# gnss-sdr/gnss-sdr

Measured on AMD Instinct MI355X. Metric: correlators/s, higher is better.
Workload: dtype f32; 1 GPU; GPS L1 C/A tracking, 32 channels/GPU x 400 epochs/block x 1400 blocks/step, fs=25 Msps, N=25000, 3-tap E/P/L, open-loop, 2 launches in flight (blocks alternate over that many banks and streams); the IF stream is RESIDENT in HBM before the timed region (host-to-device transfer excluded: pcie_inclusive is the end-to-end figure); channels_per_gpu=32, epochs_per_block=400, samples_per_epoch=25000, taps=3, stream_resident_bytes=643200000, parallelism=channels sharded over 1 GPU(s)

## Files before the change

### gnss-sdr_amd/_lib.py

```python
from __future__ import annotations

import ctypes as C
import os

_HERE = os.path.dirname(os.path.abspath(__file__))
LIB_PATH = os.environ.get("GSH_LIB_PATH") or os.path.join(_HERE, "libgnss_sdr_hip.so")

GSH_MAX_TAPS = 8
GSH_MAX_WIDE_TAPS = 64
GSH_OK = 0
GSH_ITEM_GR_COMPLEX, GSH_ITEM_SHORT, GSH_ITEM_BYTE = 0, 1, 2
GSH_ARRAY_MAX_ANTENNAS, GSH_ARRAY_MAX_BEAMS = 8, 8
GSH_ARRAY_PLANAR, GSH_ARRAY_INTERLEAVED = 0, 1
ERR_NAMES = {1: "GSH_ERR_INVALID", 2: "GSH_ERR_NO_DEVICE", 3: "GSH_ERR_HIP", 4: "GSH_ERR_STATE", 5: "GSH_ERR_UNSUPPORTED"}


class GshError(RuntimeError):
    def __init__(self, code: int, text: str):
        super().__init__(f"{ERR_NAMES.get(code, code)}: {text}")
        self.code = code


class CorrJob(C.Structure):
    _fields_ = [
# ... 161 lines not shown
        ("noise_power_estimation", C.c_float),
        ("n_segments", C.c_int32),
        ("last_filtered", C.c_int32),
        ("n_decided", C.c_uint64),
        ("n_blanked", C.c_uint64),
    ]


class CondNotch(C.Structure):
    _fields_ = [
        ("pfa", C.c_float),
        ("p_c_factor", C.c_float),
        ("length", C.c_int32),
        ("n_segments_est", C.c_int32),
        ("n_segments_reset", C.c_int32),
        ("n_segments_coeff", C.c_int32),
    ]


class CondNotchState(C.Structure):
    _fields_ = [
        ("thres", C.c_float),
        ("noise_pow_est", C.c_float),
        ("n_segments", C.c_int32),
        ("filter_state", C.c_int32),
        ("n_segments_coeff", C.c_int32),
        ("reserved", C.c_int32),
        ("z0", C.c_float * 2),
        ("n_decided", C.c_uint64),
        ("n_filtered", C.c_uint64),
    ]


class AcqResult(C.Structure):
    _fields_ = [
        ("index_time", C.c_uint32),
        ("index_doppler", C.c_uint32),
        ("doppler_hz", C.c_int32),
        ("acq_delay_samples", C.c_float),
        ("peak", C.c_float),
        ("input_power", C.c_float),
        ("second_peak", C.c_float),
        ("test_statistics", C.c_float),
    ]


_P = C.c_void_p
_F = C.POINTER(C.c_float)
_I16 = C.POINTER(C.c_int16)
_I8 = C.POINTER(C.c_int8)
SYMBOLS = {
    "gsh_abi_version": (C.c_int, []),
    "gsh_device_count": (C.c_int, []),
    "gsh_probe_read_bandwidth": (C.c_int, [C.c_int, C.c_uint64, C.c_int, C.POINTER(C.c_double)]),
    "gsh_last_error": (C.c_char_p, []),
    "gsh_device_name": (C.c_int, [C.c_int, C.c_char_p, C.c_size_t]),
    "gsh_mcorr_create": (C.c_int, [C.c_int, C.POINTER(_P)]),
    "gsh_mcorr_destroy": (None, [_P]),
    "gsh_mcorr_init": (C.c_int, [_P, C.c_int, C.c_int]),
    "gsh_mcorr_set_local_code_and_taps": (C.c_int, [_P, C.c_int, _F, _F]),
    "gsh_mcorr_set_input_output_vectors": (C.c_int, [_P, _F, _F]),
    "gsh_mcorr_set_high_dynamics_resampler": (C.c_int, [_P, C.c_int]),
    "gsh_mcorr_carrier_wipeoff_multicorrelator_resampler": (C.c_int, [_P] + [C.c_float] * 6 + [C.c_int]),
    "gsh_mcorr_carrier_wipeoff_multicorrelator_resampler6": (C.c_int, [_P] + [C.c_float] * 5 + [C.c_int]),
    "gsh_mcorr_free": (C.c_int, [_P]),
    "gsh_mcorr16_create": (C.c_int, [C.c_int, C.POINTER(_P)]),
    "gsh_mcorr16_destroy": (None, [_P]),
    "gsh_mcorr16_init": (C.c_int, [_P, C.c_int, C.c_int]),
    "gsh_mcorr16_set_local_code_and_taps": (C.c_int, [_P, C.c_int, _I16, _F]),
    "gsh_mcorr16_set_input_output_vectors": (C.c_int, [_P, _I16, _I16]),
    "gsh_mcorr16_carrier_wipeoff_multicorrelator_resampler": (C.c_int, [_P] + [C.c_float] * 4 + [C.c_int]),
    "gsh_mcorr16_free": (C.c_int, [_P]),
    "gsh_bank16_create": (C.c_int, [C.c_int, C.c_int, C.c_int, C.POINTER(_P)]),
    "gsh_bank16_destroy": (None, [_P]),
    "gsh_bank16_set_code": (C.c_int, [_P, C.c_int, _I16, C.c_int]),
    "gsh_bank16_set_stream_host": (C.c_int, [_P, _I16, C.c_uint64]),
    "gsh_bank16_set_stream_device": (C.c_int, [_P, _P, C.c_uint64]),
    "gsh_bank16_correlate": (C.c_int, [_P, C.POINTER(Corr16Job), C.c_int, _I16]),
    "gsh_bank16_upload_jobs": (C.c_int, [_P, C.POINTER(Corr16Job), C.c_int]),
    "gsh_bank16_launch": (C.c_int, [_P]),
    "gsh_bank16_read_outputs": (C.c_int, [_P, _I16, C.c_int]),
    "gsh_bank16_time_launches": (C.c_int, [_P, C.c_int, _F]),
    "gsh_bank_create": (C.c_int, [C.c_int, C.c_int, C.c_int, C.POINTER(_P)]),
    "gsh_bank_destroy": (None, [_P]),
    "gsh_bank_set_code": (C.c_int, [_P, C.c_int, _F, C.c_int]),
    "gsh_bank_set_stream_host": (C.c_int, [_P, _F, C.c_uint64]),
    "gsh_bank_set_stream_device": (C.c_int, [_P, _P, C.c_uint64]),
    "gsh_bank_correlate": (C.c_int, [_P, C.POINTER(CorrJob), C.c_int, _F]),
    "gsh_bank_upload_jobs": (C.c_int, [_P, C.POINTER(CorrJob), C.c_int]),
    "gsh_bank_launch": (C.c_int, [_P, _P]),
    "gsh_bank_synchronize": (C.c_int, [_P]),
    "gsh_bank_read_outputs": (C.c_int, [_P, _F, C.c_int]),
    "gsh_bank_time_launches": (C.c_int, [_P, C.c_int, _F]),
    "gsh_bank_set_pair_fusion": (C.c_int, [_P, C.c_int]),
    "gsh_bank_set_splits": (C.c_int, [_P, C.c_int]),
    "gsh_bank_set_sample_base": (C.c_int, [_P, C.c_uint64]),
    "gsh_bank_set_stream_ring": (C.c_int, [_P, _P]),
    "gsh_bank_correlate_wide": (C.c_int, [_P, C.POINTER(CorrJobWide), C.c_int, _F]),
    "gsh_bank_time_launches_wide": (C.c_int, [_P, C.POINTER(CorrJobWide), C.c_int, C.c_int, _F]),
    "gsh_stream_create": (C.c_int, [C.c_int, C.c_uint64, C.c_uint32, C.POINTER(_P)]),
    "gsh_stream_destroy": (None, [_P]),
    "gsh_stream_push": (C.c_int, [_P, _P, C.c_uint64, C.c_int, C.c_int, C.POINTER(C.c_uint64)]),
    "gsh_stream_push_device": (C.c_int, [_P, _P, C.c_uint64, C.c_int, C.c_int, _P, C.POINTER(C.c_uint64)]),
    "gsh_stream_push_async": (C.c_int, [_P, _P, C.c_uint64, C.c_int, C.c_int, C.POINTER(C.c_uint64)]),
    "gsh_stream_wait": (C.c_int, [_P]),
    "gsh_stream_push_staged": (C.c_int, [_P, _P, C.c_uint64, C.c_int, C.c_int, C.POINTER(C.c_uint64)]),
# ... 178 lines not shown
```

### gnss-sdr_amd/csrc/mcorr_device.h

```cpp
#ifndef GSH_MCORR_DEVICE_H
#define GSH_MCORR_DEVICE_H

#include "gsh_internal.h"
#include <cmath>
#include <type_traits>

#ifndef GSH_MC_THREADS
#define GSH_MC_THREADS 256
#endif
#define GSH_MC_NS_CAT2(a, b) a##b
#define GSH_MC_NS_CAT(a, b) GSH_MC_NS_CAT2(a, b)
#define GSH_MC_NS GSH_MC_NS_CAT(mcdev_, GSH_MC_THREADS)

namespace gsh
{
namespace GSH_MC_NS
{
constexpr int MC_THREADS = GSH_MC_THREADS;
constexpr int MC_WAVES = MC_THREADS / 64;
constexpr int MC_MARGIN = 32;
constexpr int MC_HALF_MAX_CODE_LEN = 1024;
constexpr int MC_HALF_WORDS = 2 * (MC_HALF_MAX_CODE_LEN + 2 * MC_MARGIN);
#ifndef GSH_MC_SCAN_ALL_AT_ONCE
#define GSH_MC_SCAN_ALL_AT_ONCE 1
// ... 125 lines not shown
#undef GSH_DPP_STEP
}

__device__ __forceinline__ float readlane_f(float v, int l)
{
    return __builtin_bit_cast(float, __builtin_amdgcn_readlane(__builtin_bit_cast(int, v), l));
}

__device__ __forceinline__ int floor_to_int(float x)
{
#if GSH_MC_CVT_FLR
    int k;
    asm("v_cvt_flr_i32_f32 %0, %1" : "=v"(k) : "v"(x));
    return k;
#else
    return static_cast<int>(floorf(x));
#endif
}

__device__ __forceinline__ int raw_chip_std(float step_x_n, float shift, float rem)
{
    return floor_to_int(__fsub_rn(__fadd_rn(step_x_n, shift), rem));
}

__device__ __forceinline__ int raw_chip_hd(float step, float rate, unsigned m, float shift0, float rem)
{
    const float a = __fmul_rn(step, static_cast<float>(m));
    const float q = __fmul_rn(rate, static_cast<float>(m * m));
    return floor_to_int(__fsub_rn(__fadd_rn(__fadd_rn(a, q), shift0), rem));
}

struct JobCtx
{
    int n_total;
    int n_begin;
    int n_end;
    int n_first;
    int code_len;
    float rem_carr, phase_step, phase_rate;
    float rem_code, code_step, code_rate;
    int k_lo{0}, k_hi{-1};
    int k_off{MC_MARGIN};
    bool packed{true};
    bool runs{false};
    bool aux_on{false};
    bool aux_zero{false};
    float aux_shift{0.0f};
    int aux_code_len{1};
    int aux_k_off{MC_MARGIN};
    int aux_k_lo{0}, aux_k_hi{-1};
    const float2* seed_tab{nullptr};
    const float2* fac_tab{nullptr};
};
constexpr int FAC_B = 0;
constexpr int FAC_WH = 32;
constexpr int FAC_INC = 40;
constexpr int FAC_A = 44;
constexpr int FAC_NA = 20;
constexpr int FAC_ENTRIES = 64;
static_assert(MC_THREADS > 256 || MC_THREADS / 32 <= FAC_INC - FAC_WH, "factor table: one WH entry per 32 threads");
__host__ __device__ constexpr int packed_reseed_trips(int nch) { return (GSH_MC_RESEED + nch - 1) / nch; }
template <int NCH>
__device__ __forceinline__ void fac_table_fill(float2* __restrict__ tab, float step, float rem, int n_first, int lane)
{
    const double sd = static_cast<double>(step);
    double ph;
    if (lane < FAC_WH)
        ph = static_cast<double>(2 * lane) * sd;
    else if (lane < FAC_INC)
        ph = static_cast<double>(64 * (lane - FAC_WH)) * sd;
    else if (lane < FAC_A)
        ph = (lane == FAC_INC ? 1.0 : (lane == FAC_INC + 1 ? static_cast<double>(2 * MC_THREADS) : static_cast<double>(2 * NCH * MC_THREADS))) * sd;
    else
        {
            const long long nb = static_cast<long long>(n_first) + static_cast<long long>(2 * MC_THREADS * NCH * packed_reseed_trips(NCH)) * (lane - FAC_A);
            ph = static_cast<double>(rem) + static_cast<double>(nb) * sd;
        }
    tab[lane] = expmj(ph);
}
constexpr int SEED_B = 0;
constexpr int SEED_W = 64;
constexpr int SEED_A = 80;
constexpr int SEED_INC = 82;
constexpr int SEED_ENTRIES = 88;
__device__ __forceinline__ void seed_table_fill(float2* __restrict__ tab, float step, double rem, int lane, int which)
{
    asm volatile("" : "+v"(lane));
    const double sd = static_cast<double>(step);
    if (which == 0)
        tab[SEED_B + lane] = expmj(static_cast<double>(2 * lane) * sd);
    else if (lane < 21)
        {
            double ph;
            int at;
            if (lane < 16)
                {
                    ph = static_cast<double>(128 * lane) * sd;
                    at = SEED_W + lane;
                }
            else if (lane < 18)
                {
                    ph = rem + static_cast<double>(-(lane - 16)) * sd;
                    at = SEED_A + (lane - 16);
                }
            else
                {
// ... 441 lines not shown
                    const v2f cB = lookup(aB, aux_shp, zs, aux_koff, std::false_type{});
                    pk_fma_lo(XB0, yB0, cB);
                    pk_fma_hi(XB1, yB1, cB);
                }
        }
}

struct PairedCodes
{
    v2f p, el0, el1;
};
template <bool ZP, bool KC>
__device__ __forceinline__ PairedCodes paired_codes_of(const JobCtx& c, const float* __restrict__ tab, v2f shP, v2f shL, v2f k_step_nrem, v2f nf)
{
    typedef const __attribute__((address_space(3))) float* lds_float_ptr;
    const int koff = KC ? MC_MARGIN : c.k_off;
    const v2f a = pk_mul_slo(nf, k_step_nrem);
    auto at = [&](int k, int d) -> float {
        if constexpr (KC)
            {
                unsigned byte_addr;
                asm("v_lshlrev_b32 %0, 2, %1" : "=v"(byte_addr) : "v"(k));
                return reinterpret_cast<lds_float_ptr>(byte_addr)[MC_MARGIN + d];
            }
        else
            return tab[k + koff + d];
    };
    PairedCodes d;
    {
        const v2f u = ZP ? pk_add_shi(a, k_step_nrem) : pk_add_shi(pk_add_slo(a, shP), k_step_nrem);
        d.p.x = at(floor_to_int(u.x), 0);
        d.p.y = at(floor_to_int(u.y), 0);
    }
    {
        const v2f u = pk_add_shi(pk_add_slo(a, shL), k_step_nrem);
        const int k0 = floor_to_int(u.x), k1 = floor_to_int(u.y);
        d.el0.x = at(k0, -1);
        d.el0.y = at(k0, 0);
        d.el1.x = at(k1, -1);
        d.el1.y = at(k1, 0);
    }
    return d;
}
__device__ __forceinline__ void paired_accumulate(const PairedCodes& d, v2f y0, v2f y1, v2f (&S0)[3], v2f (&S1)[3])
{
    pk_fma_lo(S0[0], y0, d.el0);
    pk_fma_lo(S1[0], y1, d.el1);
    pk_fma_lo(S0[1], y0, d.p);
    pk_fma_hi(S1[1], y1, d.p);
    pk_fma_hi(S0[2], y0, d.el0);
    pk_fma_hi(S1[2], y1, d.el1);
}

template <int NT, bool ZP, bool AUX, int NCH, int PF, bool DER = false, bool KC = false, bool MRG = false, bool HALF = false>
__device__ __forceinline__ void run_segment_packed(const JobCtx& c, const float2* __restrict__ base, const float* __restrict__ tab,
    const float (&sh)[NT], float2 (&acc)[NT], float2* acc_aux)
{
    static_assert(NCH == 1 || NCH == 2, "one or two chunks per trip");
    static_assert(!HALF || (DER && KC && !MRG), "half-chip taps: a paired-tap flavour of the whole-code table");
    constexpr int PPC = MC_PAIRS_PER_CHUNK;
    constexpr int RESEED = packed_reseed_trips(NCH);
    constexpr int TBL = 60;
    const int tid = threadIdx.x;
    const int lane = tid & 63;
    const v2f zero = {0.0f, 0.0f};
    float2 tb_b = make_float2(1.0f, 0.0f), tb_wv = tb_b, tb_a0 = tb_b, tb_inc = tb_b, tb_w = tb_b, tb_w2 = tb_b;
    if (c.seed_tab != nullptr)
        {
            int tl = tid;
            asm volatile("" : "+v"(tl));
            const float2* __restrict__ S = c.seed_tab;
            tb_b = S[SEED_B + (tl & 63)];
            tb_wv = S[SEED_W + (tl >> 6)];
            tb_a0 = S[SEED_A + (c.n_begin - c.n_first)];
            tb_inc = S[SEED_INC];
            tb_w = S[SEED_INC + 1];
            tb_w2 = S[SEED_INC + (NCH == 2 ? 2 : 1)];
        }
    const int span = c.n_end - c.n_first;
    const int n_pairs = (span + 1) >> 1;
    const int n_full = span >> 1;
    const int odd = c.n_begin - c.n_first;
    const int n_trips_all = (n_pairs + NCH * PPC - 1) / (NCH * PPC);
    int n_trips = n_trips_all;
    if constexpr (NCH == 1 || MRG)
        {
            const int left = c.n_end - (c.n_first + 128 * (tid >> 6));
            n_trips = left <= 0 ? 0 : min(n_trips_all, (left + 2 * NCH * PPC - 1) / (2 * NCH * PPC));
            n_trips = __builtin_amdgcn_readfirstlane(n_trips);
        }
    const int first_plain = odd ? 1 : 0;
    const int last_plain = n_full / (NCH * PPC);
    constexpr int TRIP = 2 * NCH * PPC;
    unsigned lane_bytes = 16u * static_cast<unsigned>(tid);
    typedef const __attribute__((address_space(1))) char* global_bytes;
    typedef float v4f_t __attribute__((ext_vector_type(4)));
    typedef const __attribute__((address_space(1))) v4f_t* global_v4f;
    typedef const __attribute__((address_space(1))) v2f* global_v2f;
    auto trip_base = [&](int i, int byte_off) -> global_bytes {
        global_bytes ub = (global_bytes)(reinterpret_cast<const char*>(base + static_cast<long long>(i) * TRIP) + byte_off);
        asm("" : "+s"(ub));
        return ub;
    };
    auto load16 = [](global_bytes p) -> float4 {
        const v4f_t v = *(global_v4f)p;
        return make_float4(v.x, v.y, v.z, v.w);
    };
    auto load8 = [](global_bytes p) -> float2 {
        const v2f v = *(global_v2f)p;
        return make_float2(v.x, v.y);
    };
    auto lane_n0 = [&](int i) -> int {
        unsigned lb = lane_bytes;
        asm volatile("" : "+v"(lb));
        return (c.n_first + i * TRIP) + static_cast<int>(lb >> 3);
    };
// ... 643 lines not shown
                epbuf[lane] = make_float4(incl.x - tot.x, incl.y - tot.y, ph.x, ph.y);
                T = make_float2(readlane_f(incl.x, 63), readlane_f(incl.y, 63));
            }
#endif
            asm volatile("" ::: "memory");

#ifdef GSH_RUNS_SKIP3
            if (false)
#else
            if (my_t < NT)
#endif
                {
                    const int k_first = chip_of(n_lo);
                    const int count = chip_of(b - 1) - k_first;
                    if (my_j == 0)
                        {
                            const float c0 = tab[k_first + c.k_off];
                            bacc.x = fmaf(c0, T.x, bacc.x);
                            bacc.y = fmaf(c0, T.y, bacc.y);
                        }
                    for (int j = my_j; j < count; j += LT)
                        {
                            const int k = k_first + 1 + j;
                            int n = static_cast<int>(ceilf(__fmul_rn(__fadd_rn(static_cast<float>(k), est_off), inv_step)));
                            n = min(max(n, n_lo + 1), b - 1);
                            while (n > n_lo + 1 && chip_of(n - 1) >= k) n--;
                            while (n < b - 1 && chip_of(n) < k) n++;
                            const int rel = n - a;
                            const int run = rel / R, pos = rel % R;
                            const float4 ep = epbuf[run];
                            const float2 qv = ybuf[run * STRIDE + max(pos - 1, 0)];
                            float2 P = make_float2(ep.x, ep.y);
                            if (pos > 0)
                                {
                                    const float2 r = cmul(qv, make_float2(ep.z, ep.w));
                                    P.x += r.x;
                                    P.y += r.y;
                                }
                            const float d = tab[k + c.k_off] - tab[k - 1 + c.k_off];
                            bacc.x = fmaf(d, T.x - P.x, bacc.x);
                            bacc.y = fmaf(d, T.y - P.y, bacc.y);
                        }
                }
            asm volatile("" ::: "memory");
        }
#pragma unroll
    for (int t = 0; t < NT; t++)
        {
            acc[t].x += (my_t == t) ? bacc.x : 0.0f;
            acc[t].y += (my_t == t) ? bacc.y : 0.0f;
        }
}

template <int NT, int MODE, bool WRAP, bool ZP = false, bool AUX = false, bool KC = false, bool PAIRK = false, bool HALFK = false>
__device__ __forceinline__ void run_segment(const JobCtx& c, const float2* __restrict__ base, const float* __restrict__ tab,
    const float (&sh)[NT], const int (&rot)[NT], float2 (&acc)[NT], float2* acc_aux = nullptr)
{
#if GSH_MC_PACKED
    if (!WRAP && MODE == 0 && c.packed && c.n_total < (1 << 24))
        {
#ifndef GSH_MC_MERGED
#define GSH_MC_MERGED 1
#endif
#ifndef GSH_MC_MERGED_BANK
#define GSH_MC_MERGED_BANK 0
#endif
            constexpr bool MRG = GSH_MC_MERGED && (MC_THREADS > 256 || GSH_MC_MERGED_BANK);
#ifdef GSH_MC_NCH
            constexpr int NCH = (NT <= 3 && !AUX) ? GSH_MC_NCH : 1;
#else
#ifdef GSH_MC_NCH_WIDE
            constexpr int NCH = (MC_THREADS <= 256 || MRG) ? 2 : 1;
#else
            constexpr int NCH = (MC_THREADS <= 256 || (MRG && NT <= 3 && !AUX)) ? 2 : 1;
#endif
#endif
#ifdef GSH_MC_PREFETCH
            constexpr int PF = GSH_MC_PREFETCH;
#else
            constexpr int PF = (MC_THREADS <= 256) ? GSH_MC_PREFETCH_BANK : GSH_MC_PREFETCH_LOOP;
#endif
            if constexpr (PAIRK && NT == 3 && ZP && !AUX && PF == 1)
                {
                    static_assert(!HALFK || (KC && NCH == 2 && !MRG), "half-chip taps: whole-code table, two chunks per trip, four accumulator sets");
                    run_segment_packed<NT, ZP, AUX, NCH, PF, true, KC, MRG, HALFK>(c, base, tab, sh, acc, acc_aux);
                    return;
                }
            run_segment_packed<NT, ZP, AUX, NCH, PF, false, KC && !HALFK, MRG>(c, base, tab, sh, acc, acc_aux);
            return;
        }
#endif
    const int tid = threadIdx.x;
    const int span = c.n_end - c.n_first;
    const int n_pairs = (span + 1) >> 1;
    const int n_full = span >> 1;
    const int odd = c.n_begin - c.n_first;
    const int n_chunks = (n_pairs + MC_PAIRS_PER_CHUNK - 1) / MC_PAIRS_PER_CHUNK;
    const int k_full_begin = odd ? 1 : 0;
    const int k_full_end = n_full / MC_PAIRS_PER_CHUNK;
    constexpr bool HDP = mode_hd_phase(MODE);

    if (odd && n_chunks > 0)
        {
            const int pair = tid;
            if (pair < n_pairs)
                {
                    const int n0 = c.n_first + 2 * pair;
                    const float2 pa = expmj(carrier_phase<HDP>(c.rem_carr, c.phase_step, c.phase_rate, n0));
                    const float2 pb = expmj(carrier_phase<HDP>(c.rem_carr, c.phase_step, c.phase_rate, n0 + 1));
                    process_pair<NT, MODE, WRAP, true, false, AUX>(c, base, tab, sh, rot, pair, pa, pb, acc, static_cast<float>(n0), acc_aux);
                }
        }

    if (k_full_end > k_full_begin)
        {
            if (HDP)
                {
                    for (int k = k_full_begin; k < k_full_end; k++)
                        {
                            const int pair = tid + k * MC_PAIRS_PER_CHUNK;
                            const int n0 = c.n_first + 2 * pair;
                            const float2 pa = expmj(carrier_phase<true>(c.rem_carr, c.phase_step, c.phase_rate, n0));
                            const float2 pb = expmj(carrier_phase<true>(c.rem_carr, c.phase_step, c.phase_rate, n0 + 1));
                            process_pair<NT, MODE, WRAP, false, false, AUX>(c, base, tab, sh, rot, pair, pa, pb, acc, static_cast<float>(n0), acc_aux);
                        }
                }
            else
                {
                    const int k_body = k_full_begin;
                    const float2 w = expmj(static_cast<double>(2 * MC_PAIRS_PER_CHUNK) * static_cast<double>(c.phase_step));
                    const float2 inc = expmj(static_cast<double>(c.phase_step));
                    for (int kb = k_body; kb < k_full_end; kb += MC_RESEED)
                        {
                            const int cnt = min(MC_RESEED, k_full_end - kb);
                            int pair = tid + kb * MC_PAIRS_PER_CHUNK;
                            float2 pa = expmj(carrier_phase<false>(c.rem_carr, c.phase_step, 0.0f, c.n_first + 2 * pair));
                            float2 pb = cmul(pa, inc);
                            float nf0 = static_cast<float>(c.n_first + 2 * pair);
#pragma unroll 2
                            for (int i = 0; i < cnt; i++)
                                {
                                    process_pair<NT, MODE, WRAP, false, ZP, AUX>(c, base, tab, sh, rot, pair, pa, pb, acc, nf0, acc_aux);
                                    pa = cmul(pa, w);
                                    pb = cmul(pb, w);
                                    pair += MC_PAIRS_PER_CHUNK;
// ... 261 lines not shown
```

### gnss-sdr_amd/csrc/multicorrelator.hip

```cpp
#include "multicorrelator.h"
#ifdef GSH_MC_VARIANT_128
#define mcorr_kernel mcorr_kernel_t128
#define mcorr_reduce_partials mcorr_reduce_partials_t128
#endif
#include "mcorr_device.h"
#include <cmath>
#include <cstdlib>

namespace gsh
{
namespace
{
using namespace mcdev;
#ifndef GSH_MC_MIN_WAVES
#define GSH_MC_MIN_WAVES 5
#endif

#ifndef GSH_MC_RUN_LEN
#define GSH_MC_RUN_LEN 8
#endif
constexpr int MC_RUN_LEN = GSH_MC_RUN_LEN;

template <int NT, int MODE, bool AUX, bool RUNS = false, bool WIN = false, bool PAIR = false, bool HALF = false>
__global__ __launch_bounds__(MC_THREADS, ((NT <= 3 && !AUX) ? GSH_MC_MIN_WAVES : 1)) void mcorr_kernel(McorrArgs a)
{
    static_assert(!PAIR || (NT == 3 && MODE == 0 && !AUX && !RUNS), "paired taps: the plain E/P/L launch");
    static_assert(!HALF || (PAIR && !WIN), "half-chip taps: a paired-tap launch with whole-code tables");
    static_assert(!RUNS || (MODE == 0 && !AUX), "the run-based path exists for the standard mode without a fused tap");
    extern __shared__ __align__(16) float lds[];
    const unsigned lb = xcd_remap(blockIdx.x, gridDim.x);
    const int slot = static_cast<int>(lb) / a.splits;
    const int split = static_cast<int>(lb) - slot * a.splits;
    const int job = a.job_list ? a.job_list[slot] : slot;
    const gsh_corr_job& J = a.jobs[job];
    const int tid = threadIdx.x;
    const int aux_job = AUX ? a.aux[job] : -1;
    if (AUX && aux_job == -2) return;

    JobCtx c;
    c.n_total = J.n_samples;
    c.code_len = a.code_lens[J.code_slot];
    c.rem_carr = J.rem_carr_phase_rad;
    c.phase_step = J.phase_step_rad;
    c.phase_rate = J.phase_rate_step_rad;
    c.rem_code = J.rem_code_phase_chips;
    c.code_step = J.code_phase_step_chips;
    c.code_rate = J.code_phase_rate_step_chips;
    c.packed = a.packed != 0;
    c.runs = RUNS && a.packed == 2;

    int seg = (c.n_total + a.splits - 1) / a.splits;
    seg = (seg + 1) & ~1;
    c.n_begin = min(split * seg, c.n_total);
    c.n_end = min(c.n_total, c.n_begin + seg);
    unsigned long long win0 = J.sample_offset + a.sample_base;
    if (a.ring_capacity) win0 %= a.ring_capacity;
    const unsigned long long abs0 = win0 + static_cast<unsigned long long>(c.n_begin);
    const int odd = static_cast<int>(abs0 & 1ULL);
// ... 194 lines not shown
                sums[2 * NT] = acc_aux.x;
                sums[2 * NT + 1] = acc_aux.y;
            }
        wave_scan_incl_n(sums);
#pragma unroll
        for (int t = 0; t < NT; t++) acc[t] = make_float2(sums[2 * t], sums[2 * t + 1]);
        if (AUX) acc_aux = make_float2(sums[2 * NT], sums[2 * NT + 1]);
    }
    const int wave = tid >> 6;
    if ((tid & 63) == 63)
        {
#pragma unroll
            for (int t = 0; t < NT; t++) red[wave * GSH_MAX_TAPS + t] = acc[t];
            if (AUX) red[wave * GSH_MAX_TAPS + NT] = acc_aux;
        }
    __syncthreads();
    if (AUX && aux_job >= 0 && tid >= GSH_MAX_TAPS && tid < 2 * GSH_MAX_TAPS)
        {
            const int tap = tid - GSH_MAX_TAPS;
            float2 s = make_float2(0.0f, 0.0f);
            if (tap == 0)
                {
#pragma unroll
                    for (int w = 0; w < MC_WAVES; w++)
                        {
                            s.x += red[w * GSH_MAX_TAPS + NT].x;
                            s.y += red[w * GSH_MAX_TAPS + NT].y;
                        }
                }
            if (a.splits == 1)
                a.out[static_cast<size_t>(aux_job) * GSH_MAX_TAPS + tap] = s;
            else
                a.partials[(static_cast<size_t>(aux_job) * a.splits + split) * GSH_MAX_TAPS + tap] = s;
        }
    if (tid < GSH_MAX_TAPS)
        {
            float2 s = make_float2(0.0f, 0.0f);
            if (tid < NT && tid < J.n_taps)
                {
#pragma unroll
                    for (int w = 0; w < MC_WAVES; w++)
                        {
                            s.x += red[w * GSH_MAX_TAPS + tid].x;
                            s.y += red[w * GSH_MAX_TAPS + tid].y;
                        }
                }
            if (a.splits == 1)
                a.out[static_cast<size_t>(job) * GSH_MAX_TAPS + tid] = s;
            else
                a.partials[(static_cast<size_t>(job) * a.splits + split) * GSH_MAX_TAPS + tid] = s;
        }
}

__global__ __launch_bounds__(256) void mcorr_reduce_partials(const float2* __restrict__ partials, float2* __restrict__ out, int n_jobs, int splits)
{
    const int i = blockIdx.x * blockDim.x + threadIdx.x;
    if (i >= n_jobs * GSH_MAX_TAPS) return;
    const int job = i / GSH_MAX_TAPS, tap = i - job * GSH_MAX_TAPS;
    float2 s = make_float2(0.0f, 0.0f);
    for (int k = 0; k < splits; k++)
        {
            const float2 p = partials[(static_cast<size_t>(job) * splits + k) * GSH_MAX_TAPS + tap];
            s.x += p.x;
            s.y += p.y;
        }
    out[i] = s;
}

template <int NT>
int launch_nt(const McorrArgs& a, int mode, size_t lds, size_t lds_half, hipStream_t stream)
{
    const dim3 grid(static_cast<unsigned>(a.n_launch) * static_cast<unsigned>(a.splits));
    const dim3 block(MC_THREADS);
    if (a.aux != nullptr)
        {
            if constexpr (NT == 3 || NT == 5)
                {
                    GSH_REQUIRE(mode == 0, "fused jobs need the standard mode");
                    if (a.window_floats > 0)
                        hipLaunchKernelGGL((mcorr_kernel<NT, 0, true, false, true>), grid, block, lds, stream, a);
                    else
                        hipLaunchKernelGGL((mcorr_kernel<NT, 0, true>), grid, block, lds, stream, a);
                    GSH_HIP(hipGetLastError());
                    return GSH_OK;
                }
            else
                return set_error(GSH_ERR_INVALID, "fused jobs exist only for the 3- and 5-tap kernels");
        }
    switch (mode)
        {
        case 0:
#ifdef GSH_MC_RUNS_EXPERIMENT
            if constexpr (NT <= 5)
                {
                    if (a.packed == 2 && a.window_floats == 0)
                        {
                            const size_t lds_runs = lds + static_cast<size_t>(MC_WAVES) * RunsLayout<MC_RUN_LEN>::FLOATS * sizeof(float);
                            if (lds_runs <= 64 * 1024)
                                {
                                    hipLaunchKernelGGL((mcorr_kernel<NT, 0, false, true>), grid, block, lds_runs, stream, a);
                                    break;
                                }
                        }
                }
#endif
            if constexpr (NT == 3)
                {
                    if (a.pair && a.packed == 1)
                        {
                            if (a.window_floats > 0)
                                hipLaunchKernelGGL((mcorr_kernel<NT, 0, false, false, true, true>), grid, block, lds, stream, a);
                            else if (a.half && lds_half > 0 && a.code_images != nullptr)
                                hipLaunchKernelGGL((mcorr_kernel<NT, 0, false, false, false, true, true>), grid, block, lds_half, stream, a);
                            else
                                hipLaunchKernelGGL((mcorr_kernel<NT, 0, false, false, false, true>), grid, block, lds, stream, a);
                            break;
                        }
                }
            if (a.window_floats > 0)
                hipLaunchKernelGGL((mcorr_kernel<NT, 0, false, false, true>), grid, block, lds, stream, a);
            else
                hipLaunchKernelGGL((mcorr_kernel<NT, 0, false>), grid, block, lds, stream, a);
            break;
        case 1:
            hipLaunchKernelGGL((mcorr_kernel<NT, 1, false>), grid, block, lds, stream, a);
            break;
        case 2:
            hipLaunchKernelGGL((mcorr_kernel<NT, 2, false>), grid, block, lds, stream, a);
            break;
        default:
            return set_error(GSH_ERR_INVALID, "unknown correlator mode %d", mode);
        }
    GSH_HIP(hipGetLastError());
    return GSH_OK;
}
}

#ifndef GSH_MC_VARIANT_128
int mcorr_packed_default()
{
    static const int v = [] {
        const char* e = std::getenv("GSH_MC_PACKED_BODY");
        if (e != nullptr && e[0] == '0') return 0;
#ifdef GSH_MC_RUNS_EXPERIMENT
        if (e != nullptr && e[0] == '2') return 2;
#endif
        if (e != nullptr && e[0] == '3') return 3;
        return 1;
    }();
    return v;
}

int mcorr_fac_default()
{
    static const int v = [] {
        const char* e = std::getenv("GSH_MC_FAC");
        return (e != nullptr && e[0] == '0') ? 0 : 1;
    }();
    return v;
}

#endif

#ifdef GSH_MC_VARIANT_128
#define mcorr_lds_bytes_window mcorr_lds_bytes_window_t128
#define mcorr_lds_bytes_fused mcorr_lds_bytes_fused_t128
// ... 83 lines not shown
    GSH_REQUIRE(args.splits >= 1, "splits must be >= 1");
    static const int class_taps[4] = {1, 3, 5, GSH_MAX_TAPS};
    for (int c = 0; c < 4; c++)
        {
            if (plan.count[c] <= 0) continue;
            McorrArgs a = args;
            a.job_list = plan.list + plan.offset[c];
            a.n_launch = plan.count[c];
            if (!plan.aux[c]) a.aux = nullptr;
#ifndef GSH_MC_VARIANT_128
            if (use_128(a, class_taps[c], mode))
                {
                    McorrClassPlan one = plan;
                    for (int o = 0; o < 4; o++)
                        if (o != c) one.count[o] = 0;
                    McorrArgs b1 = args;
                    b1.splits = args.splits;
                    const int rc1 = mcorr_launch_classes_t128(b1, one, mode, max_code_len, stream);
                    if (rc1 != GSH_OK) return rc1;
                    continue;
                }
#endif
            const size_t lds = a.aux != nullptr ? mcorr_lds_bytes_fused(max_code_len, a.window_floats)
                                                : (a.window_floats > 0 ? mcorr_lds_bytes_window(a.window_floats) : mcorr_lds_bytes(max_code_len));
            GSH_REQUIRE(lds <= 160 * 1024, "local code of %d samples does not fit the 160 KiB LDS", max_code_len);
            const size_t lds_half = mcorr_lds_bytes_half(max_code_len);
            int rc;
            switch (class_taps[c])
                {
                case 1:
                    rc = launch_nt<1>(a, mode, lds, lds_half, stream);
                    break;
                case 3:
                    rc = launch_nt<3>(a, mode, lds, lds_half, stream);
                    break;
                case 5:
                    rc = launch_nt<5>(a, mode, lds, lds_half, stream);
                    break;
                default:
                    rc = launch_nt<GSH_MAX_TAPS>(a, mode, lds, lds_half, stream);
                    break;
                }
            if (rc != GSH_OK) return rc;
        }
    if (args.splits > 1)
        {
            const int total = args.n_jobs * GSH_MAX_TAPS;
            hipLaunchKernelGGL(mcorr_reduce_partials, dim3((total + 255) / 256), dim3(256), 0, stream, args.partials, args.out, args.n_jobs, args.splits);
            GSH_HIP(hipGetLastError());
        }
    return GSH_OK;
}
}
```

### include/gnss_sdr_hip.h

```cpp
#ifndef GNSS_SDR_HIP_H
#define GNSS_SDR_HIP_H

#include <stddef.h>
#include <stdint.h>

#ifdef __cplusplus
extern "C"
{
#endif

#define GSH_ABI_VERSION 25
#define GSH_MAX_TAPS 8

    enum
    {
        GSH_OK = 0,
        GSH_ERR_INVALID = 1,
        GSH_ERR_NO_DEVICE = 2,
        GSH_ERR_HIP = 3,
        GSH_ERR_STATE = 4,
        GSH_ERR_UNSUPPORTED = 5
    };

    int gsh_abi_version(void);
    int gsh_device_count(void);
    const char* gsh_last_error(void);
    int gsh_device_name(int device, char* buf, size_t buflen);
    int gsh_probe_read_bandwidth(int device, uint64_t bytes, int reps, double* gb_per_s);

    typedef struct gsh_mcorr gsh_mcorr_t;

    int gsh_mcorr_create(int device, gsh_mcorr_t** out);
    void gsh_mcorr_destroy(gsh_mcorr_t* h);

    int gsh_mcorr_init(gsh_mcorr_t* h, int max_signal_length_samples, int n_correlators);
    int gsh_mcorr_set_local_code_and_taps(gsh_mcorr_t* h, int code_length_chips, const float* local_code_in, float* shifts_chips);
    int gsh_mcorr_set_input_output_vectors(gsh_mcorr_t* h, float* corr_out_iq, const float* sig_in_iq);
    int gsh_mcorr_set_high_dynamics_resampler(gsh_mcorr_t* h, int use_high_dynamics_resampler);
    int gsh_mcorr_carrier_wipeoff_multicorrelator_resampler(gsh_mcorr_t* h, float rem_carrier_phase_in_rad,
        float phase_step_rad, float phase_rate_step_rad, float rem_code_phase_chips, float code_phase_step_chips,
        float code_phase_rate_step_chips, int signal_length_samples);
    int gsh_mcorr_carrier_wipeoff_multicorrelator_resampler6(gsh_mcorr_t* h, float rem_carrier_phase_in_rad,
        float phase_step_rad, float rem_code_phase_chips, float code_phase_step_chips,
        float code_phase_rate_step_chips, int signal_length_samples);
    int gsh_mcorr_free(gsh_mcorr_t* h);

    typedef struct gsh_bank gsh_bank_t;

    typedef struct gsh_corr_job
    {
        uint64_t sample_offset;
        int32_t n_samples;
        int32_t code_slot;
        float rem_carr_phase_rad;
        float phase_step_rad;
        float phase_rate_step_rad;
        float rem_code_phase_chips;
        float code_phase_step_chips;
        float code_phase_rate_step_chips;
        int32_t n_taps;
        int32_t high_dyn;
        float shifts_chips[GSH_MAX_TAPS];
    } gsh_corr_job;

    int gsh_bank_create(int device, int n_code_slots, int max_code_length, gsh_bank_t** out);
    void gsh_bank_destroy(gsh_bank_t* b);
    int gsh_bank_set_code(gsh_bank_t* b, int slot, const float* code, int code_length);
    int gsh_bank_set_stream_host(gsh_bank_t* b, const float* iq, uint64_t n_samples);
    int gsh_bank_set_stream_device(gsh_bank_t* b, const void* device_iq, uint64_t n_samples);
    int gsh_bank_correlate(gsh_bank_t* b, const gsh_corr_job* jobs, int n_jobs, float* out_iq);
    int gsh_bank_set_pair_fusion(gsh_bank_t* b, int enable);
    int gsh_bank_upload_jobs(gsh_bank_t* b, const gsh_corr_job* jobs, int n_jobs);
    int gsh_bank_launch(gsh_bank_t* b, void* hip_stream);
    int gsh_bank_synchronize(gsh_bank_t* b);
    int gsh_bank_read_outputs(gsh_bank_t* b, float* out_iq, int n_jobs);
    int gsh_bank_time_launches(gsh_bank_t* b, int reps, float* avg_ms);
    int gsh_bank_set_splits(gsh_bank_t* b, int splits);
    int gsh_bank_set_sample_base(gsh_bank_t* b, uint64_t sample_base);

#define GSH_MAX_WIDE_TAPS 64
    typedef struct gsh_corr_job_wide
    {
        uint64_t sample_offset;
        int32_t n_samples;
        int32_t code_slot;
        float rem_carr_phase_rad;
        float phase_step_rad;
        float rem_code_phase_chips;
        float code_phase_step_chips;
        int32_t n_taps;
        int32_t reserved;
        float shifts_chips[GSH_MAX_WIDE_TAPS];
    } gsh_corr_job_wide;
    int gsh_bank_correlate_wide(gsh_bank_t* b, const gsh_corr_job_wide* jobs, int n_jobs, float* out_iq);
    int gsh_bank_time_launches_wide(gsh_bank_t* b, const gsh_corr_job_wide* jobs, int n_jobs, int reps, float* avg_ms);

    typedef struct gsh_mcorr16 gsh_mcorr16_t;
    int gsh_mcorr16_create(int device, gsh_mcorr16_t** out);
    void gsh_mcorr16_destroy(gsh_mcorr16_t* h);
    int gsh_mcorr16_init(gsh_mcorr16_t* h, int max_signal_length_samples, int n_correlators);
    int gsh_mcorr16_set_local_code_and_taps(gsh_mcorr16_t* h, int code_length_chips, const int16_t* local_code_in_iq, float* shifts_chips);
    int gsh_mcorr16_set_input_output_vectors(gsh_mcorr16_t* h, int16_t* corr_out_iq, const int16_t* sig_in_iq);
    int gsh_mcorr16_carrier_wipeoff_multicorrelator_resampler(gsh_mcorr16_t* h, float rem_carrier_phase_in_rad, float phase_step_rad, float rem_code_phase_chips,
        float code_phase_step_chips, int signal_length_samples);
    int gsh_mcorr16_free(gsh_mcorr16_t* h);

    typedef struct gsh_bank16 gsh_bank16_t;
    typedef struct gsh_corr16_job
    {
        uint64_t sample_offset;
        int32_t n_samples;
        int32_t code_slot;
        float rem_carr_phase_rad;
        float phase_step_rad;
        float rem_code_phase_chips;
        float code_phase_step_chips;
        int32_t n_taps;
        int32_t reserved;
        float shifts_chips[GSH_MAX_TAPS];
    } gsh_corr16_job;
    int gsh_bank16_create(int device, int n_code_slots, int max_code_length, gsh_bank16_t** out);
    void gsh_bank16_destroy(gsh_bank16_t* b);
    int gsh_bank16_set_code(gsh_bank16_t* b, int slot, const int16_t* code_iq, int code_length);
    int gsh_bank16_set_stream_host(gsh_bank16_t* b, const int16_t* iq, uint64_t n_samples);
    int gsh_bank16_set_stream_device(gsh_bank16_t* b, const void* device_iq, uint64_t n_samples);
    int gsh_bank16_correlate(gsh_bank16_t* b, const gsh_corr16_job* jobs, int n_jobs, int16_t* out_iq);
    int gsh_bank16_upload_jobs(gsh_bank16_t* b, const gsh_corr16_job* jobs, int n_jobs);
    int gsh_bank16_launch(gsh_bank16_t* b);
    int gsh_bank16_read_outputs(gsh_bank16_t* b, int16_t* out_iq, int n_jobs);
    int gsh_bank16_time_launches(gsh_bank16_t* b, int reps, float* avg_ms);
// ... 441 lines not shown
```

Before: 278.8 million correlators/s.

## Add persistent grid-stride walk kernel for half-chip 3-tap correlation jobs

Adds a persistent kernel for the 128-thread variant. It launches about one block per resident slot, taken from the occupancy query, and each block loops over jobs with a grid stride instead of one block per job. The block keeps its staged code table in LDS across consecutive jobs that use the same code slot, and raises wave priority according to how many jobs it has left. The goal is to cut block launch and teardown cost and repeated code-table staging, at the price of extra __syncthreads, a reduced set of supported job paths, and uncertain occupancy and tail balance.

```diff
diff --git a/gnss-sdr_amd/_lib.py b/gnss-sdr_amd/_lib.py
--- a/gnss-sdr_amd/_lib.py
+++ b/gnss-sdr_amd/_lib.py
@@ -237,6 +237,8 @@
 SYMBOLS = {
     "gsh_abi_version": (C.c_int, []),
     "gsh_device_count": (C.c_int, []),
+    "gsh_mcorr_walk_capacity": (C.c_int, []),
+    "gsh_mcorr_walk_launches": (C.c_uint64, []),
     "gsh_probe_read_bandwidth": (C.c_int, [C.c_int, C.c_uint64, C.c_int, C.POINTER(C.c_double)]),
     "gsh_last_error": (C.c_char_p, []),
     "gsh_device_name": (C.c_int, [C.c_int, C.c_char_p, C.c_size_t]),
diff --git a/gnss-sdr_amd/csrc/mcorr_device.h b/gnss-sdr_amd/csrc/mcorr_device.h
--- a/gnss-sdr_amd/csrc/mcorr_device.h
+++ b/gnss-sdr_amd/csrc/mcorr_device.h
@@ -201,6 +201,12 @@
     const float2* seed_tab{nullptr};
     const float2* fac_tab{nullptr};
 };
+struct JobCtxLooped : JobCtx
+{
+    int tid;
+};
+__device__ __forceinline__ int ctx_tid(const JobCtx&) { return threadIdx.x; }
+__device__ __forceinline__ int ctx_tid(const JobCtxLooped& c) { return c.tid; }
 constexpr int FAC_B = 0;
 constexpr int FAC_WH = 32;
 constexpr int FAC_INC = 40;
@@ -748,8 +754,8 @@
     pk_fma_hi(S1[2], y1, d.el1);
 }
 
-template <int NT, bool ZP, bool AUX, int NCH, int PF, bool DER = false, bool KC = false, bool MRG = false, bool HALF = false>
-__device__ __forceinline__ void run_segment_packed(const JobCtx& c, const float2* __restrict__ base, const float* __restrict__ tab,
+template <int NT, bool ZP, bool AUX, int NCH, int PF, bool DER = false, bool KC = false, bool MRG = false, bool HALF = false, typename Ctx = JobCtx>
+__device__ __forceinline__ void run_segment_packed(const Ctx& c, const float2* __restrict__ base, const float* __restrict__ tab,
     const float (&sh)[NT], float2 (&acc)[NT], float2* acc_aux)
 {
     static_assert(NCH == 1 || NCH == 2, "one or two chunks per trip");
@@ -757,7 +763,7 @@
     constexpr int PPC = MC_PAIRS_PER_CHUNK;
     constexpr int RESEED = packed_reseed_trips(NCH);
     constexpr int TBL = 60;
-    const int tid = threadIdx.x;
+    const int tid = ctx_tid(c);
     const int lane = tid & 63;
     const v2f zero = {0.0f, 0.0f};
     float2 tb_b = make_float2(1.0f, 0.0f), tb_wv = tb_b, tb_a0 = tb_b, tb_inc = tb_b, tb_w = tb_b, tb_w2 = tb_b;
@@ -1507,8 +1513,8 @@
         }
 }
 
-template <int NT, int MODE, bool WRAP, bool ZP = false, bool AUX = false, bool KC = false, bool PAIRK = false, bool HALFK = false>
-__device__ __forceinline__ void run_segment(const JobCtx& c, const float2* __restrict__ base, const float* __restrict__ tab,
+template <int NT, int MODE, bool WRAP, bool ZP = false, bool AUX = false, bool KC = false, bool PAIRK = false, bool HALFK = false, typename Ctx = JobCtx>
+__device__ __forceinline__ void run_segment(const Ctx& c, const float2* __restrict__ base, const float* __restrict__ tab,
     const float (&sh)[NT], const int (&rot)[NT], float2 (&acc)[NT], float2* acc_aux = nullptr)
 {
 #if GSH_MC_PACKED
@@ -1545,7 +1551,7 @@
             return;
         }
 #endif
-    const int tid = threadIdx.x;
+    const int tid = ctx_tid(c);
     const int span = c.n_end - c.n_first;
     const int n_pairs = (span + 1) >> 1;
     const int n_full = span >> 1;
diff --git a/gnss-sdr_amd/csrc/multicorrelator.hip b/gnss-sdr_amd/csrc/multicorrelator.hip
--- a/gnss-sdr_amd/csrc/multicorrelator.hip
+++ b/gnss-sdr_amd/csrc/multicorrelator.hip
@@ -4,6 +4,7 @@
 #define mcorr_reduce_partials mcorr_reduce_partials_t128
 #endif
 #include "mcorr_device.h"
+#include <atomic>
 #include <cmath>
 #include <cstdlib>
 
@@ -304,6 +305,196 @@
         }
 }
 
+#ifdef GSH_MC_VARIANT_128
+#ifndef GSH_MC_WALK_MIN_WAVES
+#define GSH_MC_WALK_MIN_WAVES 4
+#endif
+#ifndef GSH_MC_WALK_PRIO
+#define GSH_MC_WALK_PRIO 1
+#endif
+__global__ __launch_bounds__(MC_THREADS, GSH_MC_WALK_MIN_WAVES) void mcorr_walk_kernel_t128(McorrArgs args_in_kernarg_segment)
+{
+    constexpr int NT = 3;
+    (void)args_in_kernarg_segment;
+    typedef const __attribute__((address_space(4))) McorrArgs* kernarg_ptr;
+    typedef const __attribute__((address_space(4))) gsh_corr_job* job_ptr;
+    typedef const __attribute__((address_space(4))) int* const_int_ptr;
+    typedef const __attribute__((address_space(3))) float* lds_float_ptr;
+    extern __shared__ __align__(16) float lds[];
+    int staged = -1;
+    int tid = threadIdx.x;
+    for (unsigned slot = xcd_remap(blockIdx.x, gridDim.x);; slot += gridDim.x)
+        {
+            kernarg_ptr ap = (kernarg_ptr)__builtin_amdgcn_kernarg_segment_ptr();
+            asm volatile("" : "+s"(ap));
+#define a (*ap)
+            if (slot >= static_cast<unsigned>(a.n_launch)) break;
+#if GSH_MC_WALK_PRIO
+            {
+                const unsigned left = (static_cast<unsigned>(a.n_launch) - 1u - slot) / gridDim.x;
+                if (left >= 3u)
+                    __builtin_amdgcn_s_setprio(3);
+                else if (left == 2u)
+                    __builtin_amdgcn_s_setprio(2);
+                else if (left == 1u)
+                    __builtin_amdgcn_s_setprio(1);
+                else
+                    __builtin_amdgcn_s_setprio(0);
+            }
+#endif
+            asm volatile("" : "+v"(tid));
+            const int job = a.job_list ? ((const_int_ptr)a.job_list)[slot] : static_cast<int>(slot);
+            const job_ptr Jp = (job_ptr)a.jobs + job;
+            const int code_slot = Jp->code_slot, n_taps = Jp->n_taps;
+            const float jsh[NT] = {Jp->shifts_chips[0], Jp->shifts_chips[1], Jp->shifts_chips[2]};
+
+            JobCtxLooped c;
+            c.n_total = Jp->n_samples;
+            c.code_len = ((const_int_ptr)a.code_lens)[code_slot];
+            c.rem_carr = Jp->rem_carr_phase_rad;
+            c.phase_step = Jp->phase_step_rad;
+            c.phase_rate = Jp->phase_rate_step_rad;
+            c.rem_code = Jp->rem_code_phase_chips;
+            c.code_step = Jp->code_phase_step_chips;
+            c.code_rate = Jp->code_phase_rate_step_chips;
+            c.packed = a.packed != 0;
+            c.runs = false;
+            c.tid = tid;
+
+            c.n_begin = 0;
+            c.n_end = c.n_total;
+            unsigned long long win0 = Jp->sample_offset + a.sample_base;
+            if (a.ring_capacity) win0 %= a.ring_capacity;
+            const int odd = static_cast<int>(win0 & 1ULL);
+            c.n_first = -odd;
+            const float2* __restrict__ base = a.stream + (win0 - static_cast<unsigned long long>(odd));
+
+            const int last_tap = max(n_taps, 1) - 1;
+            float sh[NT];
+            int rot[NT];
+            sh[0] = jsh[0];
+            sh[1] = last_tap >= 1 ? jsh[1] : jsh[0];
+            sh[2] = last_tap >= 2 ? jsh[2] : sh[1];
+#pragma unroll
+            for (int t = 0; t < NT; t++) rot[t] = 0;
+
+            int lo = 0, hi = -1;
+            if (c.n_end > c.n_begin)
+                {
+                    const float smin = fminf(fminf(sh[0], sh[1]), sh[2]), smax = fmaxf(fmaxf(sh[0], sh[1]), sh[2]);
+                    lo = raw_chip_std(__fmul_rn(c.code_step, static_cast<float>(c.n_begin)), smin, c.rem_code);
+                    hi = raw_chip_std(__fmul_rn(c.code_step, static_cast<float>(c.n_end - 1)), smax, c.rem_code);
+                }
+
+            float* const tab = lds + MC_HALF_WORDS;
+            bool misfit = false;
+            int lds_floats;
+            const bool pair_ok = gsh::mcorr_half_chip_eligible(n_taps, jsh, c.code_step, Jp->high_dyn, c.code_len);
+            if (a.window_floats > 0 || !pair_ok || reinterpret_cast<size_t>((lds_float_ptr)lds) != 0)
+                {
+                    misfit = (c.n_end > c.n_begin);
+                    lds_floats = a.window_floats > 0 ? a.window_floats : c.code_len + 2 * MC_MARGIN;
+                    if (staged >= 0) __syncthreads();
+                    staged = -1;
+                }
+            else
+                {
+                    const int tab_len = c.code_len + 2 * MC_MARGIN;
+                    if (code_slot != staged)
+                        {
+                            if (staged >= 0) __syncthreads();
+                            const int rows_dbl = (2 * tab_len + 3) >> 2, rows = rows_dbl + ((tab_len + 3) >> 2);
+                            const char* const image = reinterpret_cast<const char*>(a.code_images + static_cast<size_t>(code_slot) * MCORR_HALF_IMAGE_WORDS);
+                            constexpr int PER_THREAD = (MCORR_HALF_IMAGE_WORDS / 4 + MC_THREADS - 1) / MC_THREADS;
+                            const unsigned last = 16u * static_cast<unsigned>(rows - 1), end_dbl = 16u * static_cast<unsigned>(rows_dbl);
+                            const unsigned skip = 4u * MC_HALF_WORDS - end_dbl;
+                            unsigned at[PER_THREAD];
+                            float4 row[PER_THREAD];
+                            typedef float row_t __attribute__((ext_vector_type(4)));
+                            typedef __attribute__((address_space(3))) row_t* lds_row_ptr;
+#pragma unroll
+                            for (int i = 0; i < PER_THREAD; i++)
+                                {
+                                    const unsigned r = min(16u * static_cast<unsigned>(tid + i * MC_THREADS), last);
+                                    at[i] = r < end_dbl ? r : r + skip;
+                                    row[i] = *reinterpret_cast<const float4*>(image + at[i]);
+                                }
+#pragma unroll
+                            for (int i = 0; i < PER_THREAD; i++) *reinterpret_cast<lds_row_ptr>(at[i]) = (row_t){row[i].x, row[i].y, row[i].z, row[i].w};
+                            staged = code_slot;
+                        }
+                    lds_floats = tab_len + MC_HALF_WORDS;
+                }
+            float2* red = reinterpret_cast<float2*>(lds + ((lds_floats + 3) & ~3));
+            float2* const fac = red + MC_WAVES * GSH_MAX_TAPS;
+            if (a.packed != 0 && a.fac != 0)
+                {
+                    if ((tid >> 6) == 0) fac_table_fill<2>(fac, c.phase_step, c.rem_carr, c.n_first, tid);
+                    c.fac_tab = fac;
+                }
+
+            float2 acc[NT];
+#pragma unroll
+            for (int t = 0; t < NT; t++) acc[t] = make_float2(0.0f, 0.0f);
+            float2 acc_aux = make_float2(0.0f, 0.0f);
+
+            __syncthreads();
+
+            if (misfit)
+                {
+#pragma unroll
+                    for (int t = 0; t < NT; t++) acc[t] = make_float2(__builtin_nanf(""), __builtin_nanf(""));
+                }
+            else if (c.n_end > c.n_begin)
+                {
+                    const bool fast = (c.code_step >= 0.0f) && (lo >= -MC_MARGIN) && (hi < c.code_len + MC_MARGIN) && (c.code_len >= MC_MARGIN);
+                    const bool zp = (NT == n_taps) && (sh[NT / 2] == 0.0f) && (c.n_total < (1 << 24));
+                    if (fast && zp)
+                        run_segment<NT, 0, false, true, false, true, true, true>(c, base, tab, sh, rot, acc, &acc_aux);
+                    else if (fast)
+                        run_segment<NT, 0, false, false, false, false>(c, base, tab, sh, rot, acc, &acc_aux);
+                    else
+                        run_segment<NT, 0, true, false, false>(c, base, tab, sh, rot, acc, &acc_aux);
+                }
+
+            {
+                float sums[2 * NT];
+#pragma unroll
+                for (int t = 0; t < NT; t++)
+                    {
+                        sums[2 * t] = acc[t].x;
+                        sums[2 * t + 1] = acc[t].y;
+                    }
+                wave_scan_incl_n(sums);
+#pragma unroll
+                for (int t = 0; t < NT; t++) acc[t] = make_float2(sums[2 * t], sums[2 * t + 1]);
+            }
+            const int wave = tid >> 6;
+            if ((tid & 63) == 63)
+                {
+#pragma unroll
+                    for (int t = 0; t < NT; t++) red[wave * GSH_MAX_TAPS + t] = acc[t];
+                }
+            __syncthreads();
+            if (tid < GSH_MAX_TAPS)
+                {
+                    float2 s = make_float2(0.0f, 0.0f);
+                    if (tid < NT && tid < n_taps)
+                        {
+#pragma unroll
+                            for (int w = 0; w < MC_WAVES; w++)
+                                {
+                                    s.x += red[w * GSH_MAX_TAPS + tid].x;
+                                    s.y += red[w * GSH_MAX_TAPS + tid].y;
+                                }
+                        }
+                    a.out[static_cast<size_t>(job) * GSH_MAX_TAPS + tid] = s;
+                }
+#undef a
+        }
+}
+#endif
+
 __global__ __launch_bounds__(256) void mcorr_reduce_partials(const float2* __restrict__ partials, float2* __restrict__ out, int n_jobs, int splits)
 {
     const int i = blockIdx.x * blockDim.x + threadIdx.x;
@@ -318,6 +509,48 @@
         }
     out[i] = s;
 }
+
+#ifdef GSH_MC_VARIANT_128
+int walk_capacity()
+{
+    constexpr int MAX_DEVICES = 64;
+    static std::atomic<int> cached[MAX_DEVICES];
+    int dev = 0;
+    if (hipGetDevice(&dev) != hipSuccess || dev < 0 || dev >= MAX_DEVICES) return 0;
+    int v = cached[dev].load(std::memory_order_relaxed);
+    if (v == 0)
+        {
+            const size_t lds_most = static_cast<size_t>(MC_HALF_WORDS) * sizeof(float)
+                                    + ((static_cast<size_t>(MC_HALF_MAX_CODE_LEN) + 2 * MC_MARGIN + 3) & ~static_cast<size_t>(3)) * sizeof(float)
+                                    + (MC_WAVES * GSH_MAX_TAPS + FAC_ENTRIES) * sizeof(float2);
+            int per_cu = 0, cus = 0;
+            if (hipOccupancyMaxActiveBlocksPerMultiprocessor(&per_cu, mcorr_walk_kernel_t128, MC_THREADS, lds_most) != hipSuccess
+                || hipDeviceGetAttribute(&cus, hipDeviceAttributeMultiprocessorCount, dev) != hipSuccess || per_cu <= 0 || cus <= 0)
+                {
+                    (void)hipGetLastError();
+                    v = -1;
+                }
+            else
+                v = per_cu * cus;
+            cached[dev].store(v, std::memory_order_relaxed);
+        }
+    return v > 0 ? v : 0;
+}
+
+int walk_grid(const McorrArgs& a)
+{
+    static const int forced = [] {
+        const char* e = std::getenv("GSH_MC_WALK");
+        return (e != nullptr && e[0] != '\0') ? std::atoi(e) : -1;
+    }();
+    if (forced == 0 || a.splits != 1 || a.n_launch <= 0) return 0;
+    if (forced > 0) return forced;
+    const int g = walk_capacity();
+    return (g > 0 && static_cast<long long>(a.n_launch) >= 2LL * g) ? g : 0;
+}
+
+std::atomic<unsigned long long> walk_launches{0};
+#endif
 
 template <int NT>
 int launch_nt(const McorrArgs& a, int mode, size_t lds, size_t lds_half, hipStream_t stream)
@@ -363,7 +596,18 @@
                             if (a.window_floats > 0)
                                 hipLaunchKernelGGL((mcorr_kernel<NT, 0, false, false, true, true>), grid, block, lds, stream, a);
                             else if (a.half && lds_half > 0 && a.code_images != nullptr)
-                                hipLaunchKernelGGL((mcorr_kernel<NT, 0, false, false, false, true, true>), grid, block, lds_half, stream, a);
+                                {
+#ifdef GSH_MC_VARIANT_128
+                                    const int walk = walk_grid(a);
+                                    if (walk > 0)
+                                        {
+                                            hipLaunchKernelGGL(mcorr_walk_kernel_t128, dim3(static_cast<unsigned>(walk)), block, lds_half, stream, a);
+                                            walk_launches.fetch_add(1, std::memory_order_relaxed);
+                                        }
+                                    else
+#endif
+                                        hipLaunchKernelGGL((mcorr_kernel<NT, 0, false, false, false, true, true>), grid, block, lds_half, stream, a);
+                                }
                             else
                                 hipLaunchKernelGGL((mcorr_kernel<NT, 0, false, false, false, true>), grid, block, lds, stream, a);
                             break;
@@ -553,3 +797,11 @@
     return GSH_OK;
 }
 }
+
+#ifdef GSH_MC_VARIANT_128
+extern "C"
+{
+    int gsh_mcorr_walk_capacity(void) { return gsh::walk_capacity(); }
+    uint64_t gsh_mcorr_walk_launches(void) { return gsh::walk_launches.load(std::memory_order_relaxed); }
+}
+#endif
diff --git a/include/gnss_sdr_hip.h b/include/gnss_sdr_hip.h
--- a/include/gnss_sdr_hip.h
+++ b/include/gnss_sdr_hip.h
@@ -76,6 +76,8 @@
     int gsh_bank_read_outputs(gsh_bank_t* b, float* out_iq, int n_jobs);
     int gsh_bank_time_launches(gsh_bank_t* b, int reps, float* avg_ms);
     int gsh_bank_set_splits(gsh_bank_t* b, int splits);
+    int gsh_mcorr_walk_capacity(void);
+    uint64_t gsh_mcorr_walk_launches(void);
     int gsh_bank_set_sample_base(gsh_bank_t* b, uint64_t sample_base);
 
 #define GSH_MAX_WIDE_TAPS 64
```

After: 282.5 million correlators/s, median of 6. +1.3%, better.
